# dragonlong/articulated-pose

Measured on AMD Instinct MI355X. Metric: point-clouds/sec (N=1024, eyeglasses ANCSH infer+pose-fit), higher is better.
Workload: dtype f32 (network) / f64 (joint LM)

## Files before the change

### articulated-pose_amd/csrc/pose.hip

```cpp
#include "common.h"
#include "pose_math.h"

namespace ancsh {
namespace pose {

constexpr int MODEL_A = 13;
constexpr int MODEL_B = 26;

__device__ __forceinline__ unsigned long long splitmix64(unsigned long long x) {
    x += 0x9E3779B97F4A7C15ull;
    x = (x ^ (x >> 30)) * 0xBF58476D1CE4E5B9ull;
    x = (x ^ (x >> 27)) * 0x94D049BB133111EBull;
    return x ^ (x >> 31);
}
__device__ __forceinline__ int device_draw(unsigned long long seed, int prob, int iter, int k, int n) {
    const unsigned long long h = splitmix64(seed ^ splitmix64(((unsigned long long)prob << 40) ^ ((unsigned long long)iter << 8) ^ (unsigned)k));
    return (int)(h % (unsigned long long)n);
}
enum { KEY_VALUE = 0, KEY_DSEED = 1, KEY_DKEY = 2 };
struct DKey {
    const ancsh_stream_key *key;
    int parts;
};
template <int KM> struct KeyArgT { typedef unsigned long long type; };
// ... 478 lines not shown
                load_draw3(draws, seed, prob, kbase, niter, h, 0, 3, n, d3);
                cand = d3[0] == d3[1] || d3[0] == d3[2] || d3[1] == d3[2];
            }
            const unsigned long long m = __ballot(cand);
            __syncthreads();
            if (lane == 0) wcnt[wave] = __popcll(m);
            __syncthreads();
            int start = found;
            for (int w = 0; w < wave; ++w) start += wcnt[w];
            if (cand) {
                const int slot = start + __builtin_amdgcn_mbcnt_hi((unsigned)(m >> 32), __builtin_amdgcn_mbcnt_lo((unsigned)m, 0));
                if (slot < TIE_MAX_CAND) s_cand[slot] = h;
            }
            found += wcnt[0] + wcnt[1] + wcnt[2] + wcnt[3];
        }
        __syncthreads();
        const int ncand = found < TIE_MAX_CAND ? found : TIE_MAX_CAND;
        n_near = found - ncand + (winner_degenerate ? 1 : 0);
        for (int c = 0; c < ncand; ++c) {
            const int h = s_cand[c];
            int d3[3];
            load_draw3(draws, seed, prob, kbase, niter, h, 0, 3, n, d3);
            float hs[3][3], ht[3][3], hR[9], hsc, htr[3];
#pragma unroll
            for (int i = 0; i < 3; ++i)
#pragma unroll
                for (int cc = 0; cc < 3; ++cc) {
                    hs[i][cc] = src[(size_t)(r0 + d3[i]) * 3 + cc];
                    ht[i][cc] = tgt[(size_t)(r0 + d3[i]) * 3 + cc];
                }
            estimate_single3(hs, ht, hR, hsc, htr);
            int differs = 0;
            for (int i = threadIdx.x; i < n; i += 256) {
                const float *ps = src + (size_t)(r0 + i) * 3, *pt = tgt + (size_t)(r0 + i) * 3;
                const bool f = residual_sq_f32(hR, hsc, htr, ps[0], ps[1], ps[2], pt[0], pt[1], pt[2]) < th;
                differs |= (int)(f != (out_inliers[r0 + i] != 0));
            }
            n_near += __syncthreads_or(differs) ? 1 : 0;
        }
        if ((threadIdx.x & 63) == 0) wcnt[4 + (threadIdx.x >> 6)] = n_border;
        __syncthreads();
        if (threadIdx.x == 0) {
            E.tie[prob * 2] = wcnt[4] + wcnt[5] + wcnt[6] + wcnt[7];
            E.tie[prob * 2 + 1] = winner_degenerate ? -n_near : n_near;
        }
    }
    __syncthreads();
    double Rd[9], scale, trd[3];
    if (n_in > 0) {
        refit_similarity(cs, ct, n_in, red, Rd, scale, trd);
    } else {
#pragma unroll
        for (int a = 0; a < 9; ++a) Rd[a] = NAN;
        scale = NAN; trd[0] = trd[1] = trd[2] = NAN;
    }
    if (threadIdx.x == 0) {
#pragma unroll
        for (int a = 0; a < 9; ++a) om[a] = Rd[a];
        om[9] = (double)(float)scale;
#pragma unroll
        for (int a = 0; a < 3; ++a) om[10 + a] = trd[a];
        out_best[prob * 2] = best;
        out_best[prob * 2 + 1] = best_score;
        if (E.record) {
            double *rec = E.record + (size_t)prob * 26;
#pragma unroll
            for (int a = 0; a < MODEL_A; ++a) rec[a] = om[a];
            if (E.K == 1) {
#pragma unroll
                for (int a = 0; a < MODEL_A; ++a) rec[MODEL_A + a] = om[a];
            }
        }
    }
}

struct PartFd {
    Rod b, p[3];
    double rh[3];
    double blk[6];
    double gv[3];
    double ju[3];
    double jd[3][3];

    __device__ __forceinline__ void begin(const double r[3], const double J[3]) {
        b = rod_prepare(r[0], r[1], r[2]);
#pragma unroll
        for (int q = 0; q < 3; ++q) {
            const double h = fd_step(r[q]);
            rh[q] = fast_rcp(h);
            p[q] = rod_prepare(r[0] + (q == 0 ? h : 0.0), r[1] + (q == 1 ? h : 0.0), r[2] + (q == 2 ? h : 0.0));
        }
#pragma unroll
        for (int i = 0; i < 6; ++i) blk[i] = 0.0;
        gv[0] = gv[1] = gv[2] = 0.0;
        rod_apply(b, J[0], J[1], J[2], ju[0], ju[1], ju[2]);
#pragma unroll
        for (int q = 0; q < 3; ++q) {
            double qx, qy, qz;
            rod_apply(p[q], J[0], J[1], J[2], qx, qy, qz);
            jd[0][q] = qx; jd[1][q] = qy; jd[2][q] = qz;
        }
    }
    __device__ __forceinline__ void point(double px, double py, double pz, double yx, double yy, double yz) {
        double ox, oy, oz;
        rod_apply(b, px, py, pz, ox, oy, oz);
        const double f0 = yx - ox, f1 = yy - oy, f2 = yz - oz;
        double a[3][3];
#pragma unroll
        for (int q = 0; q < 3; ++q) {
            double qx, qy, qz;
            rod_apply(p[q], px, py, pz, qx, qy, qz);
            a[0][q] = ((yx - qx) - f0) * rh[q];
            a[1][q] = ((yy - qy) - f1) * rh[q];
            a[2][q] = ((yz - qz) - f2) * rh[q];
        }
#pragma unroll
        for (int q = 0; q < 3; ++q) {
#pragma unroll
            for (int r = 0; r <= q; ++r) blk[q * (q + 1) / 2 + r] += a[0][q] * a[0][r] + a[1][q] * a[1][r] + a[2][q] * a[2][r];
            gv[q] += a[0][q] * f0 + a[1][q] * f1 + a[2][q] * f2;
        }
    }
};

__device__ __forceinline__ void assemble_normal(const PartFd &p0, const double blk0[6], const double g0[3], const PartFd &p1,
                                                const double blk1[6], const double g1[3], double wj, double A[21], double g[6]) {
    double f[3], a[3][6];
#pragma unroll
    for (int c = 0; c < 3; ++c) f[c] = p0.ju[c] - p1.ju[c];
#pragma unroll
    for (int c = 0; c < 3; ++c)
#pragma unroll
        for (int q = 0; q < 3; ++q) {
            a[c][q] = (((p0.jd[c][q] - p1.ju[c]) - f[c])) * p0.rh[q];
            a[c][3 + q] = (((p0.ju[c] - p1.jd[c][q]) - f[c])) * p1.rh[q];
        }
#pragma unroll
    for (int i = 0; i < 6; ++i) {
#pragma unroll
        for (int j = 0; j <= i; ++j) {
            double v = wj * (a[0][i] * a[0][j] + a[1][i] * a[1][j] + a[2][i] * a[2][j]);
            if (i < 3) v += blk0[i * (i + 1) / 2 + j];
            else if (j >= 3) v += blk1[(i - 3) * (i - 2) / 2 + (j - 3)];
            A[i * (i + 1) / 2 + j] = v;
        }
        g[i] = wj * (a[0][i] * f[0] + a[1][i] * f[1] + a[2][i] * f[2]) + (i < 3 ? g0[i] : g1[i - 3]);
    }
}

struct HypProblem {
    double x0[3][3], y0[3][3], x1[3][3], y1[3][3], J[3], wj;

    __device__ __forceinline__ double cost(const double x[6]) const {
        const Rod r0 = rod_prepare(x[0], x[1], x[2]), r1 = rod_prepare(x[3], x[4], x[5]);
        double s = 0.0, ox, oy, oz;
#pragma unroll
        for (int i = 0; i < 3; ++i) {
            rod_apply(r0, x0[i][0], x0[i][1], x0[i][2], ox, oy, oz);
            const double a = y0[i][0] - ox, b = y0[i][1] - oy, c = y0[i][2] - oz;
            s += a * a + b * b + c * c;
            rod_apply(r1, x1[i][0], x1[i][1], x1[i][2], ox, oy, oz);
            const double d = y1[i][0] - ox, e = y1[i][1] - oy, f = y1[i][2] - oz;
            s += d * d + e * e + f * f;
        }
        double ux, uy, uz, wx, wy, wz;
        rod_apply(r0, J[0], J[1], J[2], ux, uy, uz);
        rod_apply(r1, J[0], J[1], J[2], wx, wy, wz);
        s += wj * ((ux - wx) * (ux - wx) + (uy - wy) * (uy - wy) + (uz - wz) * (uz - wz));
        return s;
    }
    __device__ __forceinline__ void normal(const double x[6], double A[21], double g[6]) const {
        PartFd p0, p1;
        p0.begin(x, J);
#pragma unroll
        for (int i = 0; i < 3; ++i) p0.point(x0[i][0], x0[i][1], x0[i][2], y0[i][0], y0[i][1], y0[i][2]);
        p1.begin(x + 3, J);
#pragma unroll
        for (int i = 0; i < 3; ++i) p1.point(x1[i][0], x1[i][1], x1[i][2], y1[i][0], y1[i][1], y1[i][2]);
        assemble_normal(p0, p0.blk, p0.gv, p1, p1.blk, p1.gv, wj, A, g);
    }
};

__device__ __forceinline__ void scales3(const float s[3][3], const float t[3][3], float &sc, float &sc_inv) {
    double ab = 0.0, aa = 0.0, bb = 0.0;
#pragma unroll
    for (int i = 0; i < 3; ++i)
#pragma unroll
        for (int j = i + 1; j < 3; ++j) {
            double ds = 0.0, dt = 0.0;
#pragma unroll
            for (int c = 0; c < 3; ++c) {
                const double u = (double)s[i][c] - s[j][c], v = (double)t[i][c] - t[j][c];
                ds += u * u;
                dt += v * v;
            }
            ab += 2.0 * sqrt(ds) * sqrt(dt);
            aa += 2.0 * ds;
            bb += 2.0 * dt;
        }
    sc = (float)(ab / (aa + 1e-6));
    sc_inv = (float)(ab / (bb + 1e-6));
}

__device__ __forceinline__ void center_part3(const float s[3][3], const float t[3][3], float sc_inv, double xc[3][3],
                                             double yc[3][3]) {
    float sm[3], tm[3];
#pragma unroll
    for (int c = 0; c < 3; ++c) {
        sm[c] = ((s[0][c] + s[1][c]) + s[2][c]) / 3.0f;
        tm[c] = ((sc_inv * t[0][c] + sc_inv * t[1][c]) + sc_inv * t[2][c]) / 3.0f;
    }
#pragma unroll
    for (int i = 0; i < 3; ++i) {
#pragma unroll
        for (int c = 0; c < 3; ++c) {
            xc[i][c] = (double)(s[i][c] - sm[c]);
            yc[i][c] = (double)(sc_inv * t[i][c] - tm[c]);
        }
    }
}

__device__ __forceinline__ void prep_part3(const float s[3][3], const float t[3][3], float sc_inv, double xc[3][3],
                                           double yc[3][3], double rv[3]) {
    center_part3(s, t, sc_inv, xc, yc);
    double M[9] = {0, 0, 0, 0, 0, 0, 0, 0, 0};
#pragma unroll
    for (int i = 0; i < 3; ++i)
#pragma unroll
        for (int a = 0; a < 3; ++a)
#pragma unroll
            for (int b = 0; b < 3; ++b) M[a * 3 + b] += yc[i][a] * xc[i][b];
    double q[4];
    horn_quat_fast(M, q);
    quat_to_rotvec(q, rv);
}

__device__ __forceinline__ double residual_sq_f64(const double R[9], double sc, const double tr[3], float sx, float sy, float sz,
                                                  float tx, float ty, float tz) {
    const double rx = R[0] * sx + R[1] * sy + R[2] * sz, ry = R[3] * sx + R[4] * sy + R[5] * sz,
                 rz = R[6] * sx + R[7] * sy + R[8] * sz;
    const double ex = ((double)tx - sc * rx) - tr[0], ey = ((double)ty - sc * ry) - tr[1], ez = ((double)tz - sc * rz) - tr[2];
    return ex * ex + ey * ey + ez * ez;
}
__device__ __forceinline__ bool inlier_f64(const double R[9], double sc, const double tr[3], float sx, float sy, float sz,
                                           float tx, float ty, float tz, double th) {
    return residual_sq_f64(R, sc, tr, sx, sy, sz, tx, ty, tz) < th;
}

struct HypSamples {
    float s0[3][3], t0[3][3], s1[3][3], t1[3][3];
};
__device__ __forceinline__ void load_hyp_samples(const float *__restrict__ src, const float *__restrict__ tgt, const int *draws,
                                                 unsigned long long seed, int prob, int kbase, int niter, int h, int a0, int n0, int a1,
                                                 int n1, HypSamples &q) {
    int i0[3], i1[3];
    load_draw3(draws, seed, prob, kbase, niter, h, 0, 6, n0, i0);
    load_draw3(draws, seed, prob, kbase, niter, h, 3, 6, n1, i1);
#pragma unroll
    for (int i = 0; i < 3; ++i)
#pragma unroll
        for (int c = 0; c < 3; ++c) {
            q.s0[i][c] = src[(size_t)(a0 + i0[i]) * 3 + c];
            q.t0[i][c] = tgt[(size_t)(a0 + i0[i]) * 3 + c];
            q.s1[i][c] = src[(size_t)(a1 + i1[i]) * 3 + c];
            q.t1[i][c] = tgt[(size_t)(a1 + i1[i]) * 3 + c];
        }
}

template <int KM>
__global__ __launch_bounds__(64) void ransac_joint_init_kernel(const int *__restrict__ rng0, const int *__restrict__ rng1,
                                                               const float *__restrict__ src, const float *__restrict__ tgt,
                                                               int niter, const int *__restrict__ draws, KeyArg<KM> seed_arg,
                                                               double *__restrict__ scores, double *__restrict__ models) {
    const unsigned long long seed = kernel_seed<KM>(seed_arg, 1);
    const int kbase = key_problem_base<KM>(seed_arg);
    const int prob = blockIdx.y, h = blockIdx.x * 64 + threadIdx.x;
    const int a0 = rng0[prob * 2], n0 = rng0[prob * 2 + 1] - a0;
    const int a1 = rng1[prob * 2], n1 = rng1[prob * 2 + 1] - a1;
    if (h >= niter) return;
    double *mo = models + ((size_t)prob * niter + h) * MODEL_B;
    if (n0 <= 0 || n1 <= 0) {
        scores[(size_t)prob * niter + h] = -1.0;
        for (int i = 0; i < MODEL_B; ++i) mo[i] = NAN;
        return;
    }
    HypSamples q;
    load_hyp_samples(src, tgt, draws, seed, prob, kbase, niter, h, a0, n0, a1, n1, q);
    float sc0, sc0i, sc1, sc1i;
    scales3(q.s0, q.t0, sc0, sc0i);
    scales3(q.s1, q.t1, sc1, sc1i);
    double xc[3][3], yc[3][3], x[6];
    prep_part3(q.s0, q.t0, sc0i, xc, yc, x);
    prep_part3(q.s1, q.t1, sc1i, xc, yc, x + 3);
#pragma unroll
    for (int i = 0; i < 6; ++i) mo[i] = x[i];
    mo[6] = sc0i; mo[7] = sc1i; mo[8] = sc0; mo[9] = sc1;
}

constexpr int HYP_CHUNK = 256;
constexpr int HYP_CHUNK_SMALL = 64;
constexpr long HYP_SMALL_LAUNCH = 8192;
constexpr int HYP_REFILL = 16;

template <int KM>
__global__ __launch_bounds__(64) void ransac_joint_lm_kernel(const int *__restrict__ rng0, const int *__restrict__ rng1,
                                                             const float *__restrict__ src, const float *__restrict__ tgt,
                                                             const float *__restrict__ joint_dir, int niter,
                                                             const int *__restrict__ draws, KeyArg<KM> seed_arg,
                                                             double *__restrict__ models, int *__restrict__ lm_stat, int chunk) {
    const unsigned long long seed = kernel_seed<KM>(seed_arg, 1);
    const int kbase = key_problem_base<KM>(seed_arg);
    const int prob = blockIdx.y;
    const int a0 = rng0[prob * 2], n0 = rng0[prob * 2 + 1] - a0;
    const int a1 = rng1[prob * 2], n1 = rng1[prob * 2 + 1] - a1;
    if (n0 <= 0 || n1 <= 0) return;
    const int c1 = min(niter, (int)(blockIdx.x + 1) * chunk);
    int next = blockIdx.x * chunk;
    HypProblem P;
    P.J[0] = joint_dir[prob * 3]; P.J[1] = joint_dir[prob * 3 + 1]; P.J[2] = joint_dir[prob * 3 + 2];
    P.wj = 3.0;
    Lm6 S;
    bool active = false;
    int h = 0;
    for (;;) {
        const unsigned long long idle = __ballot(!active);
        const int n_idle = __popcll(idle);
        if (next < c1 && (n_idle >= HYP_REFILL || n_idle >= c1 - next || n_idle == 64)) {
            if (!active) {
                const int mine = next + __builtin_amdgcn_mbcnt_hi((unsigned)(idle >> 32), __builtin_amdgcn_mbcnt_lo((unsigned)idle, 0));
                if (mine < c1) {
                    h = mine;
                    const double *mo = models + ((size_t)prob * niter + h) * MODEL_B;
                    HypSamples q;
                    load_hyp_samples(src, tgt, draws, seed, prob, kbase, niter, h, a0, n0, a1, n1, q);
                    center_part3(q.s0, q.t0, (float)mo[6], P.x0, P.y0);
                    center_part3(q.s1, q.t1, (float)mo[7], P.x1, P.y1);
#pragma unroll
                    for (int i = 0; i < 6; ++i) S.x[i] = mo[i];
                    lm6_begin(P, S);
                    active = true;
                }
            }
            next += n_idle;
        } else if (n_idle == 64) {
            break;
        }
        if (active && lm6_trip(P, S, 1e-4, 1e-8, 1e-8, 4200)) {
            double *mo = models + ((size_t)prob * niter + h) * MODEL_B;
#pragma unroll
            for (int i = 0; i < 6; ++i) mo[i] = S.x[i];
#ifdef LM_COUNT
            if (lm_stat) { lm_stat[((size_t)prob * niter + h) * 2] = S.info | (S.trips << 4) | (S.nchol << 17); lm_stat[((size_t)prob * niter + h) * 2 + 1] = S.nfev; }
#else
            if (lm_stat) { lm_stat[((size_t)prob * niter + h) * 2] = S.info; lm_stat[((size_t)prob * niter + h) * 2 + 1] = S.nfev; }
#endif
            active = false;
        }
    }
}

constexpr int COOP_G = 8;
constexpr int COOP_XCH = 112;
constexpr int COOP_HYP_PER_WAVE = 32;

__device__ __forceinline__ void group_lds_fence() {
    __builtin_amdgcn_fence(__ATOMIC_RELEASE, "wavefront");
    __builtin_amdgcn_wave_barrier();
    __builtin_amdgcn_fence(__ATOMIC_ACQUIRE, "wavefront");
}

struct HypProblemCoop {
    double x0[3][3], y0[3][3], x1[3][3], y1[3][3], J[3], wj;
    double *xch;
    int role;

    __device__ __forceinline__ double cost(const double x[6]) const {
        const bool joint = role >= 6;
        const bool p1 = role >= 3 && role < 6;
        const int i = joint ? 0 : (p1 ? role - 3 : role);
        double partial;
        if (!joint) {
            const Rod r = p1 ? rod_prepare(x[3], x[4], x[5]) : rod_prepare(x[0], x[1], x[2]);
            const double px = p1 ? (i == 0 ? x1[0][0] : i == 1 ? x1[1][0] : x1[2][0]) : (i == 0 ? x0[0][0] : i == 1 ? x0[1][0] : x0[2][0]);
            const double py = p1 ? (i == 0 ? x1[0][1] : i == 1 ? x1[1][1] : x1[2][1]) : (i == 0 ? x0[0][1] : i == 1 ? x0[1][1] : x0[2][1]);
            const double pz = p1 ? (i == 0 ? x1[0][2] : i == 1 ? x1[1][2] : x1[2][2]) : (i == 0 ? x0[0][2] : i == 1 ? x0[1][2] : x0[2][2]);
            const double tx = p1 ? (i == 0 ? y1[0][0] : i == 1 ? y1[1][0] : y1[2][0]) : (i == 0 ? y0[0][0] : i == 1 ? y0[1][0] : y0[2][0]);
            const double ty = p1 ? (i == 0 ? y1[0][1] : i == 1 ? y1[1][1] : y1[2][1]) : (i == 0 ? y0[0][1] : i == 1 ? y0[1][1] : y0[2][1]);
            const double tz = p1 ? (i == 0 ? y1[0][2] : i == 1 ? y1[1][2] : y1[2][2]) : (i == 0 ? y0[0][2] : i == 1 ? y0[1][2] : y0[2][2]);
            double ox, oy, oz;
            rod_apply(r, px, py, pz, ox, oy, oz);
            const double a = tx - ox, b = ty - oy, c = tz - oz;
            partial = a * a + b * b + c * c;
        } else {
            const Rod r0 = rod_prepare(x[0], x[1], x[2]), r1 = rod_prepare(x[3], x[4], x[5]);
            double ux, uy, uz, wx, wy, wz;
            rod_apply(r0, J[0], J[1], J[2], ux, uy, uz);
            rod_apply(r1, J[0], J[1], J[2], wx, wy, wz);
            partial = (ux - wx) * (ux - wx) + (uy - wy) * (uy - wy) + (uz - wz) * (uz - wz);
        }
        double *cs = xch + 102;
        if (role < 7) cs[role] = partial;
        group_lds_fence();
        double s = 0.0;
#pragma unroll
        for (int k = 0; k < 3; ++k) { s += cs[k]; s += cs[3 + k]; }
        s += wj * cs[6];
        group_lds_fence();
        return s;
    }

    __device__ __forceinline__ void normal(const double x[6], double A[21], double g[6]) const {
        double *col = xch, *jdx = xch + 54, *rhx = xch + 72, *fx = xch + 78, *jux = xch + 96;
        {
            const int cr = role < 6 ? role : role - 6;
            const bool p1 = cr >= 3;
            const int q = p1 ? cr - 3 : cr;
            const double r0 = p1 ? x[3] : x[0], r1 = p1 ? x[4] : x[1], r2 = p1 ? x[5] : x[2];
            const Rod b = rod_prepare(r0, r1, r2);
            const double h = fd_step(q == 0 ? r0 : q == 1 ? r1 : r2);
            const double rh = fast_rcp(h);
            const Rod pr = rod_prepare(r0 + (q == 0 ? h : 0.0), r1 + (q == 1 ? h : 0.0), r2 + (q == 2 ? h : 0.0));
            const bool wr = role < 6;
#pragma unroll
            for (int i = 0; i < 3; ++i) {
                const double px = p1 ? x1[i][0] : x0[i][0], py = p1 ? x1[i][1] : x0[i][1], pz = p1 ? x1[i][2] : x0[i][2];
                const double yx = p1 ? y1[i][0] : y0[i][0], yy = p1 ? y1[i][1] : y0[i][1], yz = p1 ? y1[i][2] : y0[i][2];
                double ox, oy, oz, qx, qy, qz;
                rod_apply(b, px, py, pz, ox, oy, oz);
                const double f0 = yx - ox, f1 = yy - oy, f2 = yz - oz;
                rod_apply(pr, px, py, pz, qx, qy, qz);
                if (wr) {
                    col[cr * 9 + i * 3 + 0] = ((yx - qx) - f0) * rh;
                    col[cr * 9 + i * 3 + 1] = ((yy - qy) - f1) * rh;
                    col[cr * 9 + i * 3 + 2] = ((yz - qz) - f2) * rh;
                    if (q == 0) { fx[(p1 ? 9 : 0) + i * 3] = f0; fx[(p1 ? 9 : 0) + i * 3 + 1] = f1; fx[(p1 ? 9 : 0) + i * 3 + 2] = f2; }
                }
            }
            double ux, uy, uz, vx, vy, vz;
            rod_apply(b, J[0], J[1], J[2], ux, uy, uz);
            rod_apply(pr, J[0], J[1], J[2], vx, vy, vz);
            if (wr) {
                jdx[cr * 3] = vx; jdx[cr * 3 + 1] = vy; jdx[cr * 3 + 2] = vz;
                rhx[cr] = rh;
                if (q == 0) { jux[(p1 ? 3 : 0)] = ux; jux[(p1 ? 3 : 0) + 1] = uy; jux[(p1 ? 3 : 0) + 2] = uz; }
            }
        }
        group_lds_fence();
        double blk[2][6], gv[2][3];
#pragma unroll
        for (int p = 0; p < 2; ++p) {
#pragma unroll
            for (int e = 0; e < 6; ++e) blk[p][e] = 0.0;
            gv[p][0] = gv[p][1] = gv[p][2] = 0.0;
#pragma unroll
            for (int i = 0; i < 3; ++i) {
                double a[3][3];
#pragma unroll
                for (int q = 0; q < 3; ++q)
#pragma unroll
                    for (int c = 0; c < 3; ++c) a[c][q] = col[(p * 3 + q) * 9 + i * 3 + c];
                const double f0 = fx[p * 9 + i * 3], f1 = fx[p * 9 + i * 3 + 1], f2 = fx[p * 9 + i * 3 + 2];
#pragma unroll
                for (int q = 0; q < 3; ++q) {
#pragma unroll
                    for (int r = 0; r <= q; ++r) blk[p][q * (q + 1) / 2 + r] += a[0][q] * a[0][r] + a[1][q] * a[1][r] + a[2][q] * a[2][r];
                    gv[p][q] += a[0][q] * f0 + a[1][q] * f1 + a[2][q] * f2;
                }
            }
        }
        double f[3], a[3][6];
#pragma unroll
        for (int c = 0; c < 3; ++c) f[c] = jux[c] - jux[3 + c];
#pragma unroll
        for (int c = 0; c < 3; ++c)
#pragma unroll
            for (int q = 0; q < 3; ++q) {
                a[c][q] = ((jdx[q * 3 + c] - jux[3 + c]) - f[c]) * rhx[q];
                a[c][3 + q] = ((jux[c] - jdx[(3 + q) * 3 + c]) - f[c]) * rhx[3 + q];
            }
#pragma unroll
        for (int i = 0; i < 6; ++i) {
#pragma unroll
            for (int j = 0; j <= i; ++j) {
                double v = wj * (a[0][i] * a[0][j] + a[1][i] * a[1][j] + a[2][i] * a[2][j]);
                if (i < 3) v += blk[0][i * (i + 1) / 2 + j];
                else if (j >= 3) v += blk[1][(i - 3) * (i - 2) / 2 + (j - 3)];
                A[i * (i + 1) / 2 + j] = v;
            }
            g[i] = wj * (a[0][i] * f[0] + a[1][i] * f[1] + a[2][i] * f[2]) + (i < 3 ? gv[0][i] : gv[1][i - 3]);
        }
        group_lds_fence();
    }
};

template <int KM>
__global__ __launch_bounds__(64) void ransac_joint_lm_coop_kernel(const int *__restrict__ rng0, const int *__restrict__ rng1,
                                                                  const float *__restrict__ src, const float *__restrict__ tgt,
                                                                  const float *__restrict__ joint_dir, int niter,
                                                                  const int *__restrict__ draws, KeyArg<KM> seed_arg,
                                                                  double *__restrict__ models, int *__restrict__ lm_stat) {
    const unsigned long long seed = kernel_seed<KM>(seed_arg, 1);
    const int kbase = key_problem_base<KM>(seed_arg);
    __shared__ double xch[64 / COOP_G][COOP_XCH];
    const int prob = blockIdx.y, lane = threadIdx.x;
    const int a0 = rng0[prob * 2], n0 = rng0[prob * 2 + 1] - a0;
    const int a1 = rng1[prob * 2], n1 = rng1[prob * 2 + 1] - a1;
    if (n0 <= 0 || n1 <= 0) return;
    const int c1 = min(niter, (int)(blockIdx.x + 1) * COOP_HYP_PER_WAVE);
    int next = blockIdx.x * COOP_HYP_PER_WAVE;
    const int grp = lane / COOP_G;
    const unsigned long long leaders = 0x0101010101010101ull;
    HypProblemCoop P;
    P.J[0] = joint_dir[prob * 3]; P.J[1] = joint_dir[prob * 3 + 1]; P.J[2] = joint_dir[prob * 3 + 2];
    P.wj = 3.0;
    P.xch = xch[grp];
    P.role = lane & (COOP_G - 1);
    Lm6 S;
    bool active = false;
    int h = 0;
    for (;;) {
        const unsigned long long idle = __ballot(!active) & leaders;
        const int n_idle = __popcll(idle);
        if (next < c1 && n_idle > 0) {
            if (!active) {
                const int mine = next + __popcll(idle & ((1ull << (grp * COOP_G)) - 1ull));
                if (mine < c1) {
                    h = mine;
                    const double *mo = models + ((size_t)prob * niter + h) * MODEL_B;
                    HypSamples q;
                    load_hyp_samples(src, tgt, draws, seed, prob, kbase, niter, h, a0, n0, a1, n1, q);
                    center_part3(q.s0, q.t0, (float)mo[6], P.x0, P.y0);
                    center_part3(q.s1, q.t1, (float)mo[7], P.x1, P.y1);
#pragma unroll
                    for (int i = 0; i < 6; ++i) S.x[i] = mo[i];
                    lm6_begin(P, S);
                    active = true;
                }
            }
            next += n_idle;
        } else if (n_idle == 64 / COOP_G) {
            break;
        }
        if (active && lm6_trip(P, S, 1e-4, 1e-8, 1e-8, 4200)) {
            if (P.role == 0) {
                double *mo = models + ((size_t)prob * niter + h) * MODEL_B;
#pragma unroll
                for (int i = 0; i < 6; ++i) mo[i] = S.x[i];
                if (lm_stat) { lm_stat[((size_t)prob * niter + h) * 2] = S.info; lm_stat[((size_t)prob * niter + h) * 2 + 1] = S.nfev; }
            }
            active = false;
        }
    }
}

template <int KM>
__global__ __launch_bounds__(64) void ransac_joint_model_kernel(const int *__restrict__ rng0, const int *__restrict__ rng1,
                                                                const float *__restrict__ src, const float *__restrict__ tgt,
                                                                int niter, const int *__restrict__ draws, KeyArg<KM> seed_arg,
                                                                double *__restrict__ models) {
    const unsigned long long seed = kernel_seed<KM>(seed_arg, 1);
    const int kbase = key_problem_base<KM>(seed_arg);
    const int prob = blockIdx.y, h = blockIdx.x * 64 + threadIdx.x;
    const int a0 = rng0[prob * 2], n0 = rng0[prob * 2 + 1] - a0;
    const int a1 = rng1[prob * 2], n1 = rng1[prob * 2 + 1] - a1;
    if (h >= niter || n0 <= 0 || n1 <= 0) return;
    double *mo = models + ((size_t)prob * niter + h) * MODEL_B;
    HypSamples q;
    load_hyp_samples(src, tgt, draws, seed, prob, kbase, niter, h, a0, n0, a1, n1, q);
    double x[6];
#pragma unroll
    for (int i = 0; i < 6; ++i) x[i] = mo[i];
    const float sc0 = (float)mo[8], sc1 = (float)mo[9];
    double R0[9], R1[9], tr0[3], tr1[3];
    rotvec_to_mat(x, R0);
    rotvec_to_mat(x + 3, R1);
#pragma unroll
    for (int a = 0; a < 3; ++a) {
        double u = 0.0, v = 0.0;
#pragma unroll
        for (int i = 0; i < 3; ++i) {
            u += (double)q.t0[i][a] - (double)sc0 * (R0[a * 3] * q.s0[i][0] + R0[a * 3 + 1] * q.s0[i][1] + R0[a * 3 + 2] * q.s0[i][2]);
            v += (double)q.t1[i][a] - (double)sc1 * (R1[a * 3] * q.s1[i][0] + R1[a * 3 + 1] * q.s1[i][1] + R1[a * 3 + 2] * q.s1[i][2]);
        }
        tr0[a] = u / 3.0;
        tr1[a] = v / 3.0;
    }
#pragma unroll
    for (int a = 0; a < 9; ++a) { mo[a] = R0[a]; mo[13 + a] = R1[a]; }
    mo[9] = sc0; mo[22] = sc1;
#pragma unroll
    for (int a = 0; a < 3; ++a) { mo[10 + a] = tr0[a]; mo[23 + a] = tr1[a]; }
}

__global__ __launch_bounds__(256) void ransac_joint_verify_kernel(const int *__restrict__ rng0, const int *__restrict__ rng1,
                                                                 const float *__restrict__ src, const float *__restrict__ tgt,
                                                                 double th, int niter, const double *__restrict__ models,
                                                                 double *__restrict__ scores) {
    const int prob = blockIdx.y, lane = threadIdx.x & 63;
    const int h = blockIdx.x * 4 + (threadIdx.x >> 6);
    if (h >= niter) return;
    const int a0 = rng0[prob * 2], n0 = rng0[prob * 2 + 1] - a0;
    const int a1 = rng1[prob * 2], n1 = rng1[prob * 2 + 1] - a1;
    if (n0 <= 0 || n1 <= 0) return;
    const double *mo = models + ((size_t)prob * niter + h) * MODEL_B;
    double R0[9], R1[9], tr0[3], tr1[3];
#pragma unroll
    for (int a = 0; a < 9; ++a) { R0[a] = mo[a]; R1[a] = mo[13 + a]; }
    const double sc0 = mo[9], sc1 = mo[22];
#pragma unroll
    for (int a = 0; a < 3; ++a) { tr0[a] = mo[10 + a]; tr1[a] = mo[23 + a]; }
    int c0 = 0, c1 = 0;
    for (int i = lane; i < n0; i += 64) {
        const float *ps = src + (size_t)(a0 + i) * 3, *pt = tgt + (size_t)(a0 + i) * 3;
        c0 += inlier_f64(R0, sc0, tr0, ps[0], ps[1], ps[2], pt[0], pt[1], pt[2], th) ? 1 : 0;
    }
    for (int i = lane; i < n1; i += 64) {
        const float *ps = src + (size_t)(a1 + i) * 3, *pt = tgt + (size_t)(a1 + i) * 3;
        c1 += inlier_f64(R1, sc1, tr1, ps[0], ps[1], ps[2], pt[0], pt[1], pt[2], th) ? 1 : 0;
    }
#pragma unroll
    for (int o = 32; o > 0; o >>= 1) { c0 += __shfl_xor(c0, o, 64); c1 += __shfl_xor(c1, o, 64); }
    if (lane == 0) scores[(size_t)prob * niter + h] = ((double)c0 / 3.0 + (double)c1 / 3.0) / 2.0;
}

struct BlockProblem {
    const float (*x0)[3];
    const float (*y0)[3];
    const float (*x1)[3];
    const float (*y1)[3];
    int n0, n1;
    double J[3], wj;
    double *red;

    __device__ __forceinline__ double cost(const double x[6]) const {
        const Rod r0 = rod_prepare(x[0], x[1], x[2]), r1 = rod_prepare(x[3], x[4], x[5]);
        double s[1] = {0.0}, ox, oy, oz;
        for (int i = threadIdx.x; i < n0; i += 256) {
            rod_apply(r0, x0[i][0], x0[i][1], x0[i][2], ox, oy, oz);
            const double a = y0[i][0] - ox, b = y0[i][1] - oy, c = y0[i][2] - oz;
            s[0] += a * a + b * b + c * c;
        }
        for (int i = threadIdx.x; i < n1; i += 256) {
            rod_apply(r1, x1[i][0], x1[i][1], x1[i][2], ox, oy, oz);
            const double a = y1[i][0] - ox, b = y1[i][1] - oy, c = y1[i][2] - oz;
            s[0] += a * a + b * b + c * c;
        }
        block_sum<1>(s, red, 4);
        double ux, uy, uz, wx, wy, wz;
        rod_apply(r0, J[0], J[1], J[2], ux, uy, uz);
        rod_apply(r1, J[0], J[1], J[2], wx, wy, wz);
        return s[0] + wj * ((ux - wx) * (ux - wx) + (uy - wy) * (uy - wy) + (uz - wz) * (uz - wz));
    }
    __device__ __forceinline__ void normal(const double x[6], double A[21], double g[6]) const {
        PartFd p0, p1;
        p0.begin(x, J);
        for (int i = threadIdx.x; i < n0; i += 256) p0.point(x0[i][0], x0[i][1], x0[i][2], y0[i][0], y0[i][1], y0[i][2]);
        p1.begin(x + 3, J);
        for (int i = threadIdx.x; i < n1; i += 256) p1.point(x1[i][0], x1[i][1], x1[i][2], y1[i][0], y1[i][1], y1[i][2]);
        double v[18];
#pragma unroll
        for (int i = 0; i < 6; ++i) { v[i] = p0.blk[i]; v[9 + i] = p1.blk[i]; }
#pragma unroll
        for (int i = 0; i < 3; ++i) { v[6 + i] = p0.gv[i]; v[15 + i] = p1.gv[i]; }
        block_sum<18>(v, red, 4);
        assemble_normal(p0, v, v + 6, p1, v + 9, v + 15, wj, A, g);
    }
};

__device__ __forceinline__ void block_scales(const float (*cs)[3], const float (*ct)[3], int n, double *red, float &sc,
                                             float &sc_inv) {
    double pr[3] = {0, 0, 0};
    pair_sums(cs, ct, n, pr);
// ... 881 lines not shown
```

Before: 17650.

## Park long-running joint LM fits and finish them cooperatively with 32-lane groups

In the per-lane RANSAC joint LM kernel, fits that run past a trip threshold are parked in LDS slots so their lanes can pick up new hypotheses. Once no lane has a short fit left, the parked fits are finished by cooperative 32-lane groups that split the cost and normal-equation work across lanes and exchange partials through LDS. The aim is to cut the tail divergence where a few slow fits keep the whole wavefront busy. In exchange it adds LDS use, wave-level fences and serial processing of parked fits, and the cooperative path may use fewer lanes efficiently.

Result: no change. 17880, median of 6 (+1.3%).

```diff
diff --git a/articulated-pose_amd/csrc/pose.hip b/articulated-pose_amd/csrc/pose.hip
--- a/articulated-pose_amd/csrc/pose.hip
+++ b/articulated-pose_amd/csrc/pose.hip
@@ -804,6 +804,133 @@
 constexpr long HYP_SMALL_LAUNCH = 8192;
 constexpr int HYP_REFILL = 16;
 
+__device__ __forceinline__ void group_lds_fence() {
+    __builtin_amdgcn_fence(__ATOMIC_RELEASE, "wavefront");
+    __builtin_amdgcn_wave_barrier();
+    __builtin_amdgcn_fence(__ATOMIC_ACQUIRE, "wavefront");
+}
+
+constexpr int LM_PARK_TRIPS = 96;
+constexpr int LM_PARK_SLOTS = 8;
+constexpr int LM_WAVE_G = 32;
+constexpr int LM_WXCH = 136;
+
+struct ParkedFit {
+    Lm6 S;
+    HypProblem P;
+    int h;
+};
+
+struct HypProblemWave {
+    const HypProblem *pp;
+    double *xch;
+    double J[3], wj;
+    int role;
+
+    __device__ __forceinline__ double cost(const double x[6]) const {
+        const bool joint = role >= 6;
+        const bool p1 = role >= 3 && role < 6;
+        const int i = joint ? 0 : (p1 ? role - 3 : role);
+        double partial;
+        if (!joint) {
+            const Rod r = p1 ? rod_prepare(x[3], x[4], x[5]) : rod_prepare(x[0], x[1], x[2]);
+            const double(*xs)[3] = p1 ? pp->x1 : pp->x0;
+            const double(*ys)[3] = p1 ? pp->y1 : pp->y0;
+            double ox, oy, oz;
+            rod_apply(r, xs[i][0], xs[i][1], xs[i][2], ox, oy, oz);
+            const double a = ys[i][0] - ox, b = ys[i][1] - oy, c = ys[i][2] - oz;
+            partial = a * a + b * b + c * c;
+        } else {
+            const Rod r0 = rod_prepare(x[0], x[1], x[2]), r1 = rod_prepare(x[3], x[4], x[5]);
+            double ux, uy, uz, wx, wy, wz;
+            rod_apply(r0, J[0], J[1], J[2], ux, uy, uz);
+            rod_apply(r1, J[0], J[1], J[2], wx, wy, wz);
+            partial = (ux - wx) * (ux - wx) + (uy - wy) * (uy - wy) + (uz - wz) * (uz - wz);
+        }
+        double *cs = xch + 129;
+        if (role < 7) cs[role] = partial;
+        group_lds_fence();
+        double s = 0.0;
+#pragma unroll
+        for (int k = 0; k < 3; ++k) { s += cs[k]; s += cs[3 + k]; }
+        s += wj * cs[6];
+        group_lds_fence();
+        return s;
+    }
+
+    __device__ __forceinline__ void normal(const double x[6], double A[21], double g[6]) const {
+        double *col = xch, *fx = xch + 54, *jdx = xch + 72, *jux = xch + 90, *rhx = xch + 96, *out = xch + 102;
+        if (role < 6) {
+            const bool p1 = role >= 3;
+            const int q = p1 ? role - 3 : role;
+            const double(*xs)[3] = p1 ? pp->x1 : pp->x0;
+            const double(*ys)[3] = p1 ? pp->y1 : pp->y0;
+            const double r0 = p1 ? x[3] : x[0], r1 = p1 ? x[4] : x[1], r2 = p1 ? x[5] : x[2];
+            const Rod b = rod_prepare(r0, r1, r2);
+            const double h = fd_step(q == 0 ? r0 : q == 1 ? r1 : r2);
+            const double rh = fast_rcp(h);
+            const Rod pr = rod_prepare(r0 + (q == 0 ? h : 0.0), r1 + (q == 1 ? h : 0.0), r2 + (q == 2 ? h : 0.0));
+#pragma unroll
+            for (int i = 0; i < 3; ++i) {
+                const double px = xs[i][0], py = xs[i][1], pz = xs[i][2], yx = ys[i][0], yy = ys[i][1], yz = ys[i][2];
+                double ox, oy, oz, qx, qy, qz;
+                rod_apply(b, px, py, pz, ox, oy, oz);
+                const double f0 = yx - ox, f1 = yy - oy, f2 = yz - oz;
+                rod_apply(pr, px, py, pz, qx, qy, qz);
+                col[role * 9 + i * 3 + 0] = ((yx - qx) - f0) * rh;
+                col[role * 9 + i * 3 + 1] = ((yy - qy) - f1) * rh;
+                col[role * 9 + i * 3 + 2] = ((yz - qz) - f2) * rh;
+                if (q == 0) { fx[(p1 ? 9 : 0) + i * 3] = f0; fx[(p1 ? 9 : 0) + i * 3 + 1] = f1; fx[(p1 ? 9 : 0) + i * 3 + 2] = f2; }
+            }
+            double ux, uy, uz, vx, vy, vz;
+            rod_apply(b, J[0], J[1], J[2], ux, uy, uz);
+            rod_apply(pr, J[0], J[1], J[2], vx, vy, vz);
+            jdx[role * 3] = vx; jdx[role * 3 + 1] = vy; jdx[role * 3 + 2] = vz;
+            rhx[role] = rh;
+            if (q == 0) { jux[(p1 ? 3 : 0)] = ux; jux[(p1 ? 3 : 0) + 1] = uy; jux[(p1 ? 3 : 0) + 2] = uz; }
+        }
+        group_lds_fence();
+        if (role < 27) {
+            const bool is_g = role >= 21;
+            int i = is_g ? role - 21 : 0;
+            if (!is_g) while ((i + 1) * (i + 2) / 2 <= role) ++i;
+            const int j = is_g ? i : role - i * (i + 1) / 2;
+            double f[3], ai[3], aj[3];
+#pragma unroll
+            for (int c = 0; c < 3; ++c) f[c] = jux[c] - jux[3 + c];
+#pragma unroll
+            for (int c = 0; c < 3; ++c) {
+                ai[c] = i < 3 ? ((jdx[i * 3 + c] - jux[3 + c]) - f[c]) * rhx[i] : ((jux[c] - jdx[i * 3 + c]) - f[c]) * rhx[i];
+                aj[c] = j < 3 ? ((jdx[j * 3 + c] - jux[3 + c]) - f[c]) * rhx[j] : ((jux[c] - jdx[j * 3 + c]) - f[c]) * rhx[j];
+            }
+            const double *ci = col + i * 9, *cj = col + j * 9, *fp = fx + (i < 3 ? 0 : 9);
+            double v;
+            if (!is_g) {
+                v = wj * (ai[0] * aj[0] + ai[1] * aj[1] + ai[2] * aj[2]);
+                if ((i < 3) == (j < 3)) {
+                    double blk = 0.0;
+#pragma unroll
+                    for (int pt = 0; pt < 3; ++pt)
+                        blk += ci[pt * 3] * cj[pt * 3] + ci[pt * 3 + 1] * cj[pt * 3 + 1] + ci[pt * 3 + 2] * cj[pt * 3 + 2];
+                    v += blk;
+                }
+            } else {
+                double gv = 0.0;
+#pragma unroll
+                for (int pt = 0; pt < 3; ++pt) gv += ci[pt * 3] * fp[pt * 3] + ci[pt * 3 + 1] * fp[pt * 3 + 1] + ci[pt * 3 + 2] * fp[pt * 3 + 2];
+                v = wj * (ai[0] * f[0] + ai[1] * f[1] + ai[2] * f[2]) + gv;
+            }
+            out[role] = v;
+        }
+        group_lds_fence();
+#pragma unroll
+        for (int k = 0; k < 21; ++k) A[k] = out[k];
+#pragma unroll
+        for (int k = 0; k < 6; ++k) g[k] = out[21 + k];
+        group_lds_fence();
+    }
+};
+
 template <int KM>
 __global__ __launch_bounds__(64) void ransac_joint_lm_kernel(const int *__restrict__ rng0, const int *__restrict__ rng1,
                                                              const float *__restrict__ src, const float *__restrict__ tgt,
@@ -818,13 +945,28 @@
     if (n0 <= 0 || n1 <= 0) return;
     const int c1 = min(niter, (int)(blockIdx.x + 1) * chunk);
     int next = blockIdx.x * chunk;
+    __shared__ ParkedFit park[LM_PARK_SLOTS];
+    __shared__ double pxch[64 / LM_WAVE_G][LM_WXCH];
+    int n_parked = 0;
     HypProblem P;
     P.J[0] = joint_dir[prob * 3]; P.J[1] = joint_dir[prob * 3 + 1]; P.J[2] = joint_dir[prob * 3 + 2];
     P.wj = 3.0;
     Lm6 S;
     bool active = false;
-    int h = 0;
+    int h = 0, trips = 0;
     for (;;) {
+        const bool long_fit = active && trips >= LM_PARK_TRIPS;
+        const unsigned long long want = __ballot(long_fit);
+        if (want) {
+            const int k = n_parked + __builtin_amdgcn_mbcnt_hi((unsigned)(want >> 32), __builtin_amdgcn_mbcnt_lo((unsigned)want, 0));
+            if (long_fit && k < LM_PARK_SLOTS) {
+                park[k].S = S;
+                park[k].P = P;
+                park[k].h = h;
+                active = false;
+            }
+            n_parked = min(LM_PARK_SLOTS, n_parked + __popcll(want));
+        }
         const unsigned long long idle = __ballot(!active);
         const int n_idle = __popcll(idle);
         if (next < c1 && (n_idle >= HYP_REFILL || n_idle >= c1 - next || n_idle == 64)) {
@@ -841,13 +983,46 @@
                     for (int i = 0; i < 6; ++i) S.x[i] = mo[i];
                     lm6_begin(P, S);
                     active = true;
+                    trips = 0;
                 }
             }
             next += n_idle;
-        } else if (n_idle == 64) {
-            break;
-        }
-        if (active && lm6_trip(P, S, 1e-4, 1e-8, 1e-8, 4200)) {
+        }
+        const bool run = active && trips < LM_PARK_TRIPS;
+        if (__ballot(run) == 0) {
+            if (n_parked == 0) break;
+            group_lds_fence();
+            const int grp = threadIdx.x / LM_WAVE_G;
+            HypProblemWave W;
+            W.xch = pxch[grp];
+            W.role = threadIdx.x % LM_WAVE_G;
+            W.J[0] = P.J[0]; W.J[1] = P.J[1]; W.J[2] = P.J[2];
+            W.wj = P.wj;
+            for (int b = 0; b < n_parked; b += 64 / LM_WAVE_G) {
+                const int k = b + grp;
+                if (k < n_parked) {
+                    W.pp = &park[k].P;
+                    Lm6 T = park[k].S;
+                    while (!lm6_trip(W, T, 1e-4, 1e-8, 1e-8, 4200)) {}
+                    if (W.role == 0) {
+                        const int hk = park[k].h;
+                        double *mo = models + ((size_t)prob * niter + hk) * MODEL_B;
+#pragma unroll
+                        for (int i = 0; i < 6; ++i) mo[i] = T.x[i];
+#ifdef LM_COUNT
+                        if (lm_stat) { lm_stat[((size_t)prob * niter + hk) * 2] = T.info | (T.trips << 4) | (T.nchol << 17); lm_stat[((size_t)prob * niter + hk) * 2 + 1] = T.nfev; }
+#else
+                        if (lm_stat) { lm_stat[((size_t)prob * niter + hk) * 2] = T.info; lm_stat[((size_t)prob * niter + hk) * 2 + 1] = T.nfev; }
+#endif
+                    }
+                }
+                group_lds_fence();
+            }
+            n_parked = 0;
+            continue;
+        }
+        if (run) ++trips;
+        if (run && lm6_trip(P, S, 1e-4, 1e-8, 1e-8, 4200)) {
             double *mo = models + ((size_t)prob * niter + h) * MODEL_B;
 #pragma unroll
             for (int i = 0; i < 6; ++i) mo[i] = S.x[i];
@@ -864,12 +1039,6 @@
 constexpr int COOP_G = 8;
 constexpr int COOP_XCH = 112;
 constexpr int COOP_HYP_PER_WAVE = 32;
-
-__device__ __forceinline__ void group_lds_fence() {
-    __builtin_amdgcn_fence(__ATOMIC_RELEASE, "wavefront");
-    __builtin_amdgcn_wave_barrier();
-    __builtin_amdgcn_fence(__ATOMIC_ACQUIRE, "wavefront");
-}
 
 struct HypProblemCoop {
     double x0[3][3], y0[3][3], x1[3][3], y1[3][3], J[3], wj;
```
